# DTolm/VkFFT

Measured on AMD Instinct MI355X. Metric: GFLOP/s (5N log2 N) + achieved HBM GB/s, batched 1D C2C fp32, 1/2/4/8 GPU, higher is better.
Workload: dtype f32; 1 GPU; batched 1D C2C fp32 in-place, N=2^8..2^22, batch=2^27/N (1 GiB per GPU), FFT+iFFT pair per size per step (sample-0 protocol); buffer_bytes_per_gpu=1073741824, parallelism=batch-sharded x1, no collectives

## Files before the change

### vkfft_amd/csrc/kernel_pow2_pk.h

```cpp
#pragma once
#include "kernel_pow2_lean.h"
#include <utility>

namespace vkfft_mi355x {

#if defined(VKFFT_HOSTEMU)
template <typename T> struct pk2 { T x, y; };
template <typename T> inline pk2<T> operator+(pk2<T> a, pk2<T> b) { return {a.x + b.x, a.y + b.y}; }
template <typename T> inline pk2<T> operator-(pk2<T> a, pk2<T> b) { return {a.x - b.x, a.y - b.y}; }
template <typename T> inline pk2<T> operator*(pk2<T> a, pk2<T> b) { return {a.x * b.x, a.y * b.y}; }
template <typename T> inline pk2<T> operator-(pk2<T> a) { return {-a.x, -a.y}; }
template <typename V> inline V pk_xx(V a) { return V{a.x, a.x}; }
template <typename V> inline V pk_yy(V a) { return V{a.y, a.y}; }
#define VKFFT_PIN2(x) do { } while (0)
#else
template <typename T> struct pk2_of;
template <> struct pk2_of<float> { typedef float type __attribute__((ext_vector_type(2))); };
template <> struct pk2_of<double> { typedef double type __attribute__((ext_vector_type(2))); };
template <typename T> using pk2 = typename pk2_of<T>::type;
template <typename V> __device__ inline V pk_xx(V a) { return __builtin_shufflevector(a, a, 0, 0); }
template <typename V> __device__ inline V pk_yy(V a) { return __builtin_shufflevector(a, a, 1, 1); }
#define VKFFT_PIN2(x) asm volatile("" : "+v"(x))
#endif
template <typename T> __host__ __device__ inline pk2<T> pk_splat(T s) { return pk2<T>{s, s}; }

#if defined(VKFFT_HOSTEMU)
#define VKFFT_PKPROF_DECL do { } while (0)
#define VKFFT_PKPROF(i) do { } while (0)
#define VKFFT_PKPROF_FLUSH() do { } while (0)
#else
#define VKFFT_PKPROF_DECL __shared__ unsigned long long spc[12]; unsigned long long ptk = 0; if constexpr ((MODE & 4) != 0) { if (threadIdx.x < 12) spc[threadIdx.x] = 0; ptk = __builtin_readcyclecounter(); }
#define VKFFT_PKPROF(i) do { if constexpr ((MODE & 4) != 0) { if (threadIdx.x == 0) { const unsigned long long now = __builtin_readcyclecounter(); spc[i] += now - ptk; ptk = now; } } } while (0)
#define VKFFT_PKPROF_FLUSH() do { if constexpr ((MODE & 4) != 0) { if (threadIdx.x == 0 && p.prof) { for (int i = 0; i < 12; i++) p.prof[(size_t)blockIdx.x * 12 + i] = spc[i]; } } } while (0)
#endif

template <typename T> struct cxp { pk2<T> re, im; };
template <typename T> __device__ inline cxp<T> pcadd(cxp<T> a, cxp<T> b) { return {a.re + b.re, a.im + b.im}; }
template <typename T> __device__ inline cxp<T> pcsub(cxp<T> a, cxp<T> b) { return {a.re - b.re, a.im - b.im}; }
template <typename T> __device__ inline cxp<T> pcmul1(cxp<T> a, pk2<T> w) {
	const pk2<T> wx = pk_xx(w), wy = pk_yy(w);
	return {a.re * wx - a.im * wy, a.re * wy + a.im * wx};
}
template <typename T> __device__ inline cxp<T> pcmul2(cxp<T> a, pk2<T> wre, pk2<T> wim) { return {a.re * wre - a.im * wim, a.re * wim + a.im * wre}; }

#if defined(VKFFT_HOSTEMU)
template <typename T> inline pk2<T> pk_cmul_aos(pk2<T> a, pk2<T> b) { return {a.x * b.x - a.y * b.y, a.x * b.y + a.y * b.x}; }
#else
template <typename T> __device__ inline pk2<T> pk_cmul_aos(pk2<T> a, pk2<T> b) {
	const pk2<T> br = __builtin_shufflevector(b, -b, 3, 0);
	return pk_xx(a) * b + pk_yy(a) * br;
}
#endif

template <int R, typename T> __device__ inline void pk_dif_inplace(cxp<T>* x) {
#pragma unroll
	for (int h = R / 2; h >= 1; h >>= 1) {
#pragma unroll
		for (int blk = 0; blk < R; blk += 2 * h) {
#pragma unroll
			for (int j = 0; j < h; j++) {
				const cxp<T> a = x[blk + j], b = x[blk + j + h];
				x[blk + j] = pcadd(a, b);
				const int kk = j * (16 / h);
				if (kk == 0) x[blk + j + h] = pcsub(a, b);
				else if (kk == 8) x[blk + j + h] = cxp<T>{a.im - b.im, b.re - a.re};
				else {
					const cxp<T> d = pcsub(a, b);
					const pk2<T> c = pk_splat<T>((T)pow2_cos32(kk)), s = pk_splat<T>((T)pow2_sin32(kk));
					x[blk + j + h] = cxp<T>{d.re * c + d.im * s, d.im * c - d.re * s};
				}
			}
		}
		VKFFT_SCHED_FENCE();
	}
}

template <typename T, typename TW> __device__ inline pk2<T> pk_tw(const TW& lut, uint32_t s, uint32_t constOff) { const cx<T> w = lut.get(s, constOff); return pk2<T>{w.x, w.y}; }

template <typename T, typename SCH, int SI, int TPF, typename TW, int TWG>
__device__ inline void pk_lean_butterflies(cxp<T>* v, const TW lut, const uint32_t tau) {
	constexpr int LOGE = SCH::LOGE, E = 1 << LOGE;
	constexpr int LOGR = SCH::bits[SI], R = 1 << LOGR, NB = E / R;
	constexpr int LOGS = SCH::logS(SI), S = 1 << LOGS;
#pragma unroll
	for (int b = 0; b < NB; b++) {
		if constexpr (SI > 0) {
			const uint32_t s = (tau + b * TPF) & (S - 1);
			constexpr int LO = SCH::lutOff(SI);
#pragma unroll
			for (int i0 = 1; i0 < R; i0 += TWG) {
				const int i1 = i0 + TWG < R ? i0 + TWG : R;
				pk2<T> w[TWG];
#pragma unroll
				for (int i = i0; i < i1; i++) w[i - i0] = pk_tw<T>(lut, s, (uint32_t)(LO + (i - 1) * S));
				VKFFT_SCHED_FENCE();
#pragma unroll
				for (int i = i0; i < i1; i++) { cxp<T>& q = v[b + i * NB]; q = pcmul1(q, w[i - i0]); VKFFT_PIN2(q.re); VKFFT_PIN2(q.im); }
				VKFFT_SCHED_FENCE();
			}
		}
		cxp<T> x[R];
#pragma unroll
		for (int i = 0; i < R; i++) x[i] = v[b + i * NB];
		pk_dif_inplace<R, T>(x);
#pragma unroll
		for (int k = 0; k < R; k++) v[b + k * NB] = x[pow2_bitrev(k, LOGR)];
	}
}

template <typename T, typename SCH, int SI, int TPF, int TC, int PART>
__device__ inline void pk_lean_exchange_part(cxp<T>* v, T* plane, const uint32_t tau) {
	constexpr int LOGE = SCH::LOGE, E = 1 << LOGE, P = SCH::bits[0];
	constexpr int LOGR = SCH::bits[SI], R = 1 << LOGR, NB = E / R;
	constexpr int LOGS = SCH::logS(SI), S = 1 << LOGS;
	static_assert(TC > 0 && TC % 2 == 0, "column tiles of even width");
#pragma unroll
	for (int b = 0; b < NB; b++) {
		const uint32_t t = tau + b * TPF;
		const uint32_t s = t & (S - 1);
		const uint32_t ob = ((t - s) << LOGR) + s;
		T* const wp = plane + pow2_lean_slot<TC, P>(ob);
#pragma unroll
		for (int k = 0; k < R; k++) *(pk2<T>*)(wp + pow2_lean_step<TC, P>(k * S)) = PART ? v[b + k * NB].im : v[b + k * NB].re;
	}
	VKFFT_SYNC();
	const T* const rp = plane + pow2_lean_slot<TC, P>(tau);
#pragma unroll
	for (int m = 0; m < E; m++) {
		const pk2<T> r = *(const pk2<T>*)(rp + pow2_lean_step<TC, P>(m * TPF));
		if (PART) v[m].im = r; else v[m].re = r;
	}
}

template <typename T, typename SCH, int SI, int TPF, int TC, typename TW, int TWG>
__device__ inline void pk_lean_stages(cxp<T>* v, T* plane, const TW lut, const uint32_t tau) {
	pk_lean_butterflies<T, SCH, SI, TPF, TW, TWG>(v, lut, tau);
	if constexpr (SI + 1 < SCH::NS) {
		pk_lean_exchange_part<T, SCH, SI, TPF, TC, 0>(v, plane, tau);
		VKFFT_SYNC();
		pk_lean_exchange_part<T, SCH, SI, TPF, TC, 1>(v, plane, tau);
		if constexpr (SI + 2 < SCH::NS) VKFFT_SYNC();
		pk_lean_stages<T, SCH, SI + 1, TPF, TC, TW, TWG>(v, plane, lut, tau);
	}
}

template <typename T, int L, int E, int TPF, int TC, int NT>
__device__ inline void pk_lean_transpose(const cxp<T>* v, cxp<T>* r, T* plane, const uint32_t tid, const uint32_t c, const uint32_t tau) {
	constexpr int PT = L + 64 / TC;
	static_assert(E * NT * 2 == L * TC && (PT % 2) == 0, "two columns per thread");
#pragma unroll
	for (int part = 0; part < 2; part++) {
		if (part) VKFFT_SYNC();
		T* const w0 = plane + c * PT + tau;
#pragma unroll
		for (int m = 0; m < E; m++) { const pk2<T> q = part ? v[m].im : v[m].re; w0[m * TPF] = q.x; w0[PT + m * TPF] = q.y; }
		VKFFT_SYNC();
#pragma unroll
		for (int i = 0; i < E; i++) {
			const uint32_t idx = tid + i * NT;
			const uint32_t kp = idx % (L / 2), cc = idx / (L / 2);
			const pk2<T> pr = *(const pk2<T>*)(plane + cc * PT + 2u * kp);
			if (part) r[i].im = pr; else r[i].re = pr;
		}
	}
}

#if defined(VKFFT_HOSTEMU)
template <typename T> struct pk4 { T x, y, z, w; };
template <typename T, int AUX> inline pk4<T> gb_load_aos2(GBuf b, uint32_t voff, uint32_t soff) {
	if (voff >= kGbRange) return pk4<T>{(T)0, (T)0, (T)0, (T)0};
	const T* q = (const T*)(b.base + (uint64_t)voff + soff);
	return pk4<T>{q[0], q[1], q[2], q[3]};
}
template <typename T> inline cxp<T> pk_from_aos(pk4<T> t) { return cxp<T>{{t.x, t.z}, {t.y, t.w}}; }
template <typename T, int AUX> inline void gb_store_aos2(GBuf b, uint32_t voff, cxp<T> v) {
	if (voff >= kGbRange) return;
	T* q = (T*)(b.base + (uint64_t)voff);
	q[0] = v.re.x; q[1] = v.im.x; q[2] = v.re.y; q[3] = v.im.y;
}
template <typename T, int E> inline void gb_landed_raw(pk4<T>*) { }
template <typename T, int AUX> inline cxp<T> gb_load_soa2(GBuf b, uint32_t voff, uint32_t soff) {
	if (voff >= kGbRange) return cxp<T>{{(T)0, (T)0}, {(T)0, (T)0}};
	const T* q = (const T*)(b.base + (uint64_t)voff + soff);
	return cxp<T>{{q[0], q[1]}, {q[2], q[3]}};
}
template <typename T, int AUX> inline void gb_store_soa2(GBuf b, uint32_t voff, cxp<T> v) {
	if (voff >= kGbRange) return;
	T* q = (T*)(b.base + (uint64_t)voff);
	q[0] = v.re.x; q[1] = v.re.y; q[2] = v.im.x; q[3] = v.im.y;
}
template <typename T, int E> inline void gb_landed_pk(cxp<T>*) { }
#else
template <typename T> struct pk4_of;
template <> struct pk4_of<float> { typedef float type __attribute__((ext_vector_type(4))); };
template <typename T> using pk4 = typename pk4_of<T>::type;
template <typename T, int AUX> __device__ inline pk4<T> gb_load_aos2(GBuf b, uint32_t voff, uint32_t soff) {
	static_assert(sizeof(T) == 4, "pairs of fp32 complex only");
	return __builtin_bit_cast(pk4<T>, __builtin_amdgcn_raw_buffer_load_b128(b.r, voff, soff, AUX));
}
template <typename T> __device__ inline cxp<T> pk_from_aos(pk4<T> t) {
	T a = t.y, b = t.z;
	asm("v_swap_b32 %0, %1" : "+v"(a), "+v"(b));
	return cxp<T>{pk2<T>{t.x, a}, pk2<T>{b, t.w}};
}
template <typename T, int AUX> __device__ inline void gb_store_aos2(GBuf b, uint32_t voff, cxp<T> v) {
	static_assert(sizeof(T) == 4, "pairs of fp32 complex only");
	T a = v.re.y, c = v.im.x;
	asm("v_swap_b32 %0, %1" : "+v"(a), "+v"(c));
	const pk4<T> t = {v.re.x, a, c, v.im.y};
	__builtin_amdgcn_raw_buffer_store_b128(__builtin_bit_cast(vk_u32x4, t), b.r, voff, 0, AUX);
}
template <typename T, int E> __device__ inline void gb_landed_raw(pk4<T>* v) {
#pragma unroll
	for (int m = 0; m < E; m++) asm volatile("" : "+v"(v[m]));
}
template <typename T, int AUX> __device__ inline cxp<T> gb_load_soa2(GBuf b, uint32_t voff, uint32_t soff) {
	static_assert(sizeof(T) == 4, "pairs of fp32 complex only");
	const vk_u32x4 t = __builtin_amdgcn_raw_buffer_load_b128(b.r, voff, soff, AUX);
	return cxp<T>{pk2<T>{__uint_as_float(t.x), __uint_as_float(t.y)}, pk2<T>{__uint_as_float(t.z), __uint_as_float(t.w)}};
}
template <typename T, int AUX> __device__ inline void gb_store_soa2(GBuf b, uint32_t voff, cxp<T> v) {
	static_assert(sizeof(T) == 4, "pairs of fp32 complex only");
	vk_u32x4 t; t.x = __float_as_uint(v.re.x); t.y = __float_as_uint(v.re.y); t.z = __float_as_uint(v.im.x); t.w = __float_as_uint(v.im.y);
	__builtin_amdgcn_raw_buffer_store_b128(t, b.r, voff, 0, AUX);
}
template <typename T, int E> __device__ inline void gb_landed_pk(cxp<T>* v) {
#pragma unroll
	for (int m = 0; m < E; m++) asm volatile("" : "+v"(v[m].re), "+v"(v[m].im));
}
#endif

template <typename T> struct RowGlobal {
	GBuf tab;
	__device__ inline cxp<T> get(uint32_t tau, uint32_t constK) const { return gb_load_soa2<T, 0>(tab, tau * 16u, constK * 16u); }
};
template <typename T> struct RowLds {
	const cx<T>* tab;
	__device__ inline cxp<T> get(uint32_t tau, uint32_t constK) const {
#if defined(VKFFT_HOSTEMU)
		const T* q = (const T*)(tab + 2u * (tau + constK));
		return cxp<T>{{q[0], q[1]}, {q[2], q[3]}};
#else
		const pk4<T> t = *(const pk4<T>*)(tab + 2u * (tau + constK));
		return cxp<T>{pk2<T>{t.x, t.y}, pk2<T>{t.z, t.w}};
#endif
	}
};
template <typename T, int LOGE> struct PkFsTw {
	static constexpr int HIB = (LOGE + 1) / 2, LOB = LOGE - HIB, NA = 1 << HIB, NB = (1 << LOB) - 1;
	pk2<T> lo[NA + NB], hi[NA + NB];
};
template <typename T, int LOGE, int TPF>
__device__ inline void pk_fs_request(PkFsTw<T, LOGE>& q, const GBuf gtab, const uint32_t fsLoBits, const uint32_t tau, const uint32_t colEven) {
	constexpr uint32_t ES = (uint32_t)sizeof(cx<T>);
	constexpr int LOB = PkFsTw<T, LOGE>::LOB, NA = PkFsTw<T, LOGE>::NA, NB = PkFsTw<T, LOGE>::NB;
	const uint32_t loMask = (1u << fsLoBits) - 1u;
	const uint32_t hiBase = (loMask + 1u) * ES;
	auto ld = [&](uint32_t voff, uint32_t soff) { const cx<T> w = gb_load<T>(gtab, voff, soff); return pk2<T>{w.x, w.y}; };
#pragma unroll
	for (int j = 0; j < NA + NB; j++) {
		const uint32_t e = (j < NA ? tau + (uint32_t)((j << LOB) * TPF) : (uint32_t)((j - NA + 1) * TPF)) * colEven;
		q.lo[j] = ld((e & loMask) * ES, 0); q.hi[j] = ld((e >> fsLoBits) * ES, hiBase);
	}
}
template <typename T, int LOGE, int TPF, typename ROW>
__device__ inline void pk_fs_apply(cxp<T>* v, const PkFsTw<T, LOGE>& q, const ROW row, const uint32_t tau, const pk2<T>* hiStep = nullptr) {
	constexpr int E = 1 << LOGE;
	constexpr int LOB = PkFsTw<T, LOGE>::LOB, NA = PkFsTw<T, LOGE>::NA, NB = PkFsTw<T, LOGE>::NB;
	pk2<T> A[NA], B[NB + 1];
#pragma unroll
	for (int j = 0; j < NA; j++) { A[j] = pk_cmul_aos<T>(q.lo[j], q.hi[j]); if (hiStep) A[j] = pk_cmul_aos<T>(A[j], *hiStep); }
	B[0] = pk2<T>{(T)1, (T)0};
#pragma unroll
	for (int i = 1; i <= NB; i++) B[i] = pk_cmul_aos<T>(q.lo[NA + i - 1], q.hi[NA + i - 1]);
	constexpr int CH = 4;
#pragma unroll
	for (int m0 = 0; m0 < E; m0 += CH) {
		cxp<T> uv[CH];
#pragma unroll
		for (int i = 0; i < CH; i++) uv[i] = row.get(tau, (uint32_t)((m0 + i) * TPF));
		VKFFT_SCHED_FENCE();
#pragma unroll
		for (int i = 0; i < CH; i++) {
			const int m = m0 + i;
			const pk2<T> w0 = (m & ((1 << LOB) - 1)) ? pk_cmul_aos<T>(A[m >> LOB], B[m & ((1 << LOB) - 1)]) : A[m >> LOB];
			const pk2<T> w0x = pk_xx(w0), w0y = pk_yy(w0);
			v[m] = pcmul2(v[m], w0x * uv[i].re - w0y * uv[i].im, w0y * uv[i].re + w0x * uv[i].im);
			VKFFT_PIN2(v[m].re); VKFFT_PIN2(v[m].im);
		}
		VKFFT_SCHED_FENCE();
	}
}

#if defined(VKFFT_HOSTEMU)
template <typename T> inline pk2<T> pka_cmul(pk2<T> a, pk2<T> w) { return {a.x * w.x - a.y * w.y, a.y * w.x + a.x * w.y}; }
template <typename T> inline pk2<T> pka_cmul_const(pk2<T> d, T c, T s) { return {d.x * c + d.y * s, d.y * c - d.x * s}; }
template <typename T> inline pk2<T> pka_sub_mi(pk2<T> a, pk2<T> b) { return {a.y - b.y, b.x - a.x}; }
#else
template <typename T> __device__ inline pk2<T> pka_cmul(pk2<T> a, pk2<T> w) {
	if constexpr (sizeof(T) == 4) {
		const pk2<T> t = a * pk_xx(w);
		pk2<T> r;
		asm("v_pk_fma_f32 %0, %1, %2, %3 op_sel:[1,1,0] op_sel_hi:[0,1,1] neg_lo:[1,0,0]" : "=v"(r) : "v"(a), "v"(w), "v"(t));
		return r;
	} else return pk2<T>{a.x * w.x - a.y * w.y, a.y * w.x + a.x * w.y};
}
template <typename T> __device__ inline pk2<T> pka_cmul_const(pk2<T> d, T c, T s) {
	if constexpr (sizeof(T) == 4) {
		const pk2<T> t = d * pk_splat<T>(c), ss = pk_splat<T>(s);
		pk2<T> r;
		asm("v_pk_fma_f32 %0, %1, %2, %3 op_sel:[1,0,0] op_sel_hi:[0,1,1] neg_hi:[1,0,0]" : "=v"(r) : "v"(d), "s"(ss), "v"(t));
		return r;
	} else return pk2<T>{d.x * c + d.y * s, d.y * c - d.x * s};
}
template <typename T> __device__ inline pk2<T> pka_sub_mi(pk2<T> a, pk2<T> b) {
	if constexpr (sizeof(T) == 4) {
		pk2<T> r;
		asm("v_pk_add_f32 %0, %1, %2 op_sel:[1,1] op_sel_hi:[0,0] neg_lo:[0,1] neg_hi:[1,0]" : "=v"(r) : "v"(a), "v"(b));
		return r;
	} else return pk2<T>{a.y - b.y, b.x - a.x};
}
#endif

template <typename F, int... I> __host__ __device__ inline void vk_static_for_impl(F&& f, std::integer_sequence<int, I...>) { (f(std::integral_constant<int, I>{}), ...); }
template <int N, typename F> __host__ __device__ inline void vk_static_for(F&& f) { vk_static_for_impl(f, std::make_integer_sequence<int, N>{}); }
constexpr int vk_ilog2(int n) { int l = 0; while ((1 << l) < n) l++; return l; }

template <int R, typename T> __device__ inline void pka_dif_inplace(pk2<T>* x) {
	vk_static_for<vk_ilog2(R)>([&](auto li) {
		constexpr int h = (R / 2) >> decltype(li)::value;
		vk_static_for<R / 2>([&](auto bi) {
			constexpr int blk = (decltype(bi)::value / h) * 2 * h, j = decltype(bi)::value % h;
			const pk2<T> a = x[blk + j], b = x[blk + j + h];
			x[blk + j] = a + b;
			constexpr int kk = j * (16 / h);
			if constexpr (kk == 0) x[blk + j + h] = a - b;
			else if constexpr (kk == 8) x[blk + j + h] = pka_sub_mi<T>(a, b);
			else x[blk + j + h] = pka_cmul_const<T>(a - b, (T)pow2_cos32(kk), (T)pow2_sin32(kk));
		});
		VKFFT_SCHED_FENCE();
	});
}

template <typename T, typename SCH, int SI, int TPF, typename TW, int TWG>
__device__ inline void pka_lean_butterflies(pk2<T>* v, const TW lut, const uint32_t tau) {
	constexpr int LOGE = SCH::LOGE, E = 1 << LOGE;
	constexpr int LOGR = SCH::bits[SI], R = 1 << LOGR, NB = E / R;
	constexpr int LOGS = SCH::logS(SI), S = 1 << LOGS;
#pragma unroll
	for (int b = 0; b < NB; b++) {
		if constexpr (SI > 0) {
			const uint32_t s = (tau + b * TPF) & (S - 1);
			constexpr int LO = SCH::lutOff(SI);
#pragma unroll
			for (int i0 = 1; i0 < R; i0 += TWG) {
				const int i1 = i0 + TWG < R ? i0 + TWG : R;
				pk2<T> w[TWG];
#pragma unroll
				for (int i = i0; i < i1; i++) w[i - i0] = pk_tw<T>(lut, s, (uint32_t)(LO + (i - 1) * S));
				VKFFT_SCHED_FENCE();
#pragma unroll
				for (int i = i0; i < i1; i++) { pk2<T>& q = v[b + i * NB]; q = pka_cmul<T>(q, w[i - i0]); VKFFT_PIN2(q); }
				VKFFT_SCHED_FENCE();
			}
		}
		pk2<T> x[R];
#pragma unroll
		for (int i = 0; i < R; i++) x[i] = v[b + i * NB];
		pka_dif_inplace<R, T>(x);
#pragma unroll
		for (int k = 0; k < R; k++) v[b + k * NB] = x[pow2_bitrev(k, LOGR)];
	}
}
template <typename T, typename SCH, int SI, int TPF, int PART, bool WAVE>
__device__ inline void pka_lean_exchange_part(pk2<T>* v, T* plane, const uint32_t tau) {
	constexpr int LOGE = SCH::LOGE, E = 1 << LOGE, P = SCH::bits[0];
	constexpr int LOGR = SCH::bits[SI], R = 1 << LOGR, NB = E / R;
	constexpr int LOGS = SCH::logS(SI), S = 1 << LOGS;
#pragma unroll
	for (int b = 0; b < NB; b++) {
		const uint32_t t = tau + b * TPF;
		const uint32_t s = t & (S - 1);
		const uint32_t ob = ((t - s) << LOGR) + s;
		T* const wp = plane + pow2_lean_slot<0, P>(ob);
#pragma unroll
		for (int k = 0; k < R; k++) wp[pow2_lean_step<0, P>(k * S)] = PART ? v[b + k * NB].y : v[b + k * NB].x;
	}
	if constexpr (WAVE) VKFFT_WAVE_SYNC(); else VKFFT_SYNC();
	const T* const rp = plane + pow2_lean_slot<0, P>(tau);
#pragma unroll
	for (int m = 0; m < E; m++) {
		const T r = rp[pow2_lean_step<0, P>(m * TPF)];
		if (PART) v[m].y = r; else v[m].x = r;
	}
}
template <typename T, typename SCH, int SI, int TPF, typename TW, int TWG, bool WAVE = false>
__device__ inline void pka_lean_stages(pk2<T>* v, T* plane, const TW lut, const uint32_t tau) {
	pka_lean_butterflies<T, SCH, SI, TPF, TW, TWG>(v, lut, tau);
	if constexpr (SI + 1 < SCH::NS) {
		pka_lean_exchange_part<T, SCH, SI, TPF, 0, WAVE>(v, plane, tau);
		if constexpr (WAVE) VKFFT_WAVE_SYNC(); else VKFFT_SYNC();
		pka_lean_exchange_part<T, SCH, SI, TPF, 1, WAVE>(v, plane, tau);
		if constexpr (SI + 2 < SCH::NS) { if constexpr (WAVE) VKFFT_WAVE_SYNC(); else VKFFT_SYNC(); }
		pka_lean_stages<T, SCH, SI + 1, TPF, TW, TWG, WAVE>(v, plane, lut, tau);
	}
}

template <typename T, typename SCH, int WPE, int TWG, int FPW = 1>
__global__ void __launch_bounds__(((1 << SCH::LOGN) >> SCH::LOGE) * FPW, WPE) pow2_row_lean_pk_kernel(const PassParams p) {
	constexpr int LOGN = SCH::LOGN, N = 1 << LOGN, LOGE = SCH::LOGE, E = 1 << LOGE, TPF = N / E;
	constexpr uint32_t ES = (uint32_t)sizeof(cx<T>);
	constexpr int PL = (int)pow2_lean_plane_elems<SCH, 0>();
	__shared__ T planes[FPW * PL];
	const uint32_t tau = FPW > 1 ? threadIdx.x % (uint32_t)TPF : threadIdx.x, fl = FPW > 1 ? threadIdx.x / (uint32_t)TPF : 0u;
	T* const plane = planes + fl * PL;
	uint32_t wg = p.reverseTiles ? gridDim.x - 1u - blockIdx.x : blockIdx.x;
	const uint32_t f0 = (wg % p.tilesPerG0) * (uint32_t)FPW + fl;
	wg /= p.tilesPerG0;
	const uint32_t g1 = wg % p.dim[1].count, g2 = wg / p.dim[1].count;
	const bool valid = FPW == 1 || f0 < p.dim[0].count;
	const GBuf gin = make_gbuf((const cx<T>*)p.in + ((int64_t)g1 * p.dim[1].inStride + (int64_t)g2 * p.dim[2].inStride + (int64_t)(FPW == 1 ? f0 : f0 - fl) * p.dim[0].inStride));
	const GBuf gout = make_gbuf((cx<T>*)p.out + ((int64_t)g1 * p.dim[1].outStride + (int64_t)g2 * p.dim[2].outStride + (int64_t)(FPW == 1 ? f0 : f0 - fl) * p.dim[0].outStride));
	const GBuf glut = make_gbuf(p.lut);
	const uint32_t laneIn = !valid ? kGbInvalid : (tau + (FPW == 1 ? 0u : fl * (uint32_t)p.dim[0].inStride)) * ES;
	const uint32_t laneOut = !valid ? kGbInvalid : (tau + (FPW == 1 ? 0u : fl * (uint32_t)p.dim[0].outStride)) * ES;
	pk2<T> v[E];
	auto ld = [&](uint32_t voff, uint32_t soff) { const cx<T> q = gb_load<T>(gin, voff, soff); return pk2<T>{q.x, q.y}; };
	if (p.padInN) {
#pragma unroll
		for (int m = 0; m < E; m++) v[m] = ld((tau + (uint32_t)(m * TPF) - p.padInL < p.padInN) ? kGbInvalid : laneIn, (uint32_t)(m * TPF) * ES);
	} else {
#pragma unroll
		for (int m = 0; m < E; m++) v[m] = ld(laneIn, (uint32_t)(m * TPF) * ES);
	}
	if (p.swapIn) {
#pragma unroll
		for (int m = 0; m < E; m++) v[m].y = -v[m].y;
	}
	pka_lean_stages<T, SCH, 0, TPF, TwGlobal<T>, TWG, false>(v, plane, TwGlobal<T>{glut}, tau);
	const T sc = (T)p.scale;
	if (sc != (T)1 || p.swapOut) {
		const pk2<T> f = {sc, p.swapOut ? -sc : sc};
#pragma unroll
		for (int m = 0; m < E; m++) v[m] = v[m] * f;
	}
	if (p.padOutN) {
#pragma unroll
		for (int m = 0; m < E; m++) gb_store<T>(gout, (tau + (uint32_t)(m * TPF) - p.padOutL < p.padOutN) ? kGbInvalid : laneOut, (uint32_t)(m * TPF) * ES, cx<T>{v[m].x, v[m].y});
	} else {
#pragma unroll
		for (int m = 0; m < E; m++) gb_store<T>(gout, laneOut, (uint32_t)(m * TPF) * ES, cx<T>{v[m].x, v[m].y});
	}
}
template <typename T, typename SCH, int WPE, int TWG, int FPW = 1> void pow2_row_lean_pk_launch(const PassParams& prm, dim3 grid, hipStream_t s) {
	hipLaunchKernelGGL((pow2_row_lean_pk_kernel<T, SCH, WPE, TWG, FPW>), grid, dim3(((1 << SCH::LOGN) >> SCH::LOGE) * FPW), 0, s, prm);
}

template <typename T, typename SCH, int TWG>
__global__ void __launch_bounds__((1 << SCH::LOGN) >> SCH::LOGE, 2) pow2_row_pairs_kernel(const PassParams p) {
	constexpr int LOGN2 = SCH::LOGN, N2 = 1 << LOGN2, LOGE = SCH::LOGE, E = 1 << LOGE, TPF = N2 / E, H = E / 2;
	constexpr uint32_t ES = (uint32_t)sizeof(cx<T>);
	typedef Pow2Sched<SCH::bits[0], SCH::bits[1], SCH::bits[2], 1> SF;
	constexpr int LUTC = SF::lutOff(3);
	static_assert(SCH::bits[3] == 0 && sizeof(T) == 4, "three stages on pairs of fp32 samples");
	__shared__ __attribute__((aligned(16))) T plane[pow2_lean_plane_elems<SCH, 2>()];
	const uint32_t tau = threadIdx.x;
	const uint32_t total = p.tilesPerG0 * p.dim[1].count * p.dim[2].count;
	const GBuf glut = make_gbuf(p.lut);
	pk4<T> ra[H], rb[H];
	auto rowBase = [&](uint32_t w, bool out) -> int64_t {
		uint32_t wg = p.reverseTiles ? total - 1u - w : w;
		const uint32_t f0 = wg % p.tilesPerG0; wg /= p.tilesPerG0;
		const uint32_t g1 = wg % p.dim[1].count, g2 = wg / p.dim[1].count;
		return out ? (int64_t)g1 * p.dim[1].outStride + (int64_t)g2 * p.dim[2].outStride + (int64_t)f0 * p.dim[0].outStride
		           : (int64_t)g1 * p.dim[1].inStride + (int64_t)g2 * p.dim[2].inStride + (int64_t)f0 * p.dim[0].inStride;
	};
	auto request = [&](uint32_t w, int h, pk4<T>* raw) {
		VKFFT_OPAQUE_ZERO(oq);
		const bool live = w < total;
		const GBuf gin = make_gbuf((const cx<T>*)p.in + (live ? rowBase(w, false) : 0));
		const uint32_t lane = live ? tau * 2u * ES + oq : kGbInvalid;
#pragma unroll
		for (int m = 0; m < H; m++) raw[m] = gb_load_aos2<T, 0>(gin, lane, (uint32_t)((h * H + m) * TPF) * 2u * ES);
	};
	uint32_t w = blockIdx.x;
	request(w, 0, ra);
	request(w, 1, rb);
	for (; w < total; w += gridDim.x) {
		cxp<T> v[E];
#pragma unroll
		for (int m = 0; m < H; m++) v[m] = pk_from_aos<T>(ra[m]);
#pragma unroll
		for (int m = 0; m < H; m++) v[H + m] = pk_from_aos<T>(rb[m]);
		if (p.swapIn) {
#pragma unroll
			for (int m = 0; m < E; m++) v[m].im = -v[m].im;
		}
		request(w + gridDim.x, 0, ra);
		pk_lean_stages<T, SCH, 0, TPF, 2, TwGlobal<T>, TWG>(v, plane, TwGlobal<T>{glut}, tau);
		VKFFT_SYNC();
		const T sc = (T)p.scale, sci = p.swapOut ? -sc : sc;
		const GBuf gout = make_gbuf((cx<T>*)p.out + rowBase(w, true));
		VKFFT_OPAQUE_ZERO(oz);
		const uint32_t lane = tau * ES + oz;
		constexpr int CH = 8;
#pragma unroll
		for (int m0 = 0; m0 < E; m0 += CH) {
			pk2<T> tw[CH];
#pragma unroll
			for (int i = 0; i < CH; i++) tw[i] = pk_tw<T>(TwGlobal<T>{glut}, tau, (uint32_t)(LUTC + (m0 + i) * TPF));
			VKFFT_SCHED_FENCE();
#pragma unroll
			for (int i = 0; i < CH; i++) {
				const int m = m0 + i;
				const T tr = v[m].re.y * tw[i].x - v[m].im.y * tw[i].y, ti = v[m].re.y * tw[i].y + v[m].im.y * tw[i].x;
				const cx<T> lo = {(v[m].re.x + tr) * sc, (v[m].im.x + ti) * sci}, hi = {(v[m].re.x - tr) * sc, (v[m].im.x - ti) * sci};
				gb_store<T>(gout, lane, (uint32_t)(m * TPF) * ES, lo);
				gb_store<T>(gout, lane, (uint32_t)(m * TPF + N2) * ES, hi);
			}
			VKFFT_SCHED_FENCE();
		}
		request(w + gridDim.x, 1, rb);
	}
}
template <typename T, typename SCH, int TWG> void pow2_row_pairs_launch(const PassParams& prm, dim3 grid, hipStream_t s) {
	const unsigned resident = pow2_num_cus();
	hipLaunchKernelGGL((pow2_row_pairs_kernel<T, SCH, TWG>), dim3(grid.x < resident ? grid.x : resident), dim3((1 << SCH::LOGN) >> SCH::LOGE), 0, s, prm);
}

}
```

### vkfft_amd/csrc/kernels_pow2.hip

```cpp
#include "engine.h"
#include "kernel_pow2.h"
#include "kernel_pow2_pk.h"
#include <cstdio>
#include <cstdlib>

namespace vkfft_mi355x {


template <typename T, typename SCH, int FPW> void pow2_row_launch(const PassParams& prm, dim3 grid, hipStream_t s) {
	constexpr int threads = ((1 << SCH::LOGN) >> SCH::LOGE) * FPW;
	hipLaunchKernelGGL((pow2_row_kernel<T, SCH, FPW>), grid, dim3(threads), 0, s, prm);
}

template <typename T, typename SCH, int TC> void pow2_col_launch(const PassParams& prm, dim3 grid, hipStream_t s) {
	constexpr int threads = ((1 << SCH::LOGN) >> SCH::LOGE) * TC;
	if (prm.bigSpan) hipLaunchKernelGGL((pow2_col_kernel<T, SCH, TC, true>), grid, dim3(threads), 0, s, prm);
	else hipLaunchKernelGGL((pow2_col_kernel<T, SCH, TC, false>), grid, dim3(threads), 0, s, prm);
}

#define VKFFT_P2C(T, dp, b0, b1, b2, b3, tc) \
	{ (b0) + (b1) + (b2) + (b3), dp, {b0, b1, b2, b3}, tc, (((1 << ((b0) + (b1) + (b2) + (b3))) >> Pow2Sched<b0, b1, b2, b3>::LOGE) * (tc)), &pow2_col_launch<T, Pow2Sched<b0, b1, b2, b3>, tc> }

#define VKFFT_P2(T, dp, b0, b1, b2, b3, fpw) \
	{ (b0) + (b1) + (b2) + (b3), dp, {b0, b1, b2, b3}, fpw, (((1 << ((b0) + (b1) + (b2) + (b3))) >> Pow2Sched<b0, b1, b2, b3>::LOGE) * (fpw)), &pow2_row_launch<T, Pow2Sched<b0, b1, b2, b3>, fpw> }

#define VKFFT_P2L(T, dp, b0, b1, b2, b3, wpe, twg, pfn) \
	{ (b0) + (b1) + (b2) + (b3), dp, {b0, b1, b2, b3}, 1, ((1 << ((b0) + (b1) + (b2) + (b3))) >> Pow2Sched<b0, b1, b2, b3>::LOGE), &pow2_row_lean_launch<T, Pow2Sched<b0, b1, b2, b3>, wpe, twg, pfn>, "pow2_row_lean_kernel" }

#define VKFFT_P2K(T, dp, b0, b1, b2, b3, wpe, twg) \
	{ (b0) + (b1) + (b2) + (b3), dp, {b0, b1, b2, b3}, 1, ((1 << ((b0) + (b1) + (b2) + (b3))) >> Pow2Sched<b0, b1, b2, b3>::LOGE), &pow2_row_lean_pk_launch<T, Pow2Sched<b0, b1, b2, b3>, wpe, twg>, "pow2_row_lean_pk_kernel" }

#define VKFFT_P2KF(T, dp, b0, b1, b2, b3, wpe, twg, fpw) \
	{ (b0) + (b1) + (b2) + (b3), dp, {b0, b1, b2, b3}, fpw, ((1 << ((b0) + (b1) + (b2) + (b3))) >> Pow2Sched<b0, b1, b2, b3>::LOGE) * (fpw), &pow2_row_lean_pk_launch<T, Pow2Sched<b0, b1, b2, b3>, wpe, twg, fpw>, "pow2_row_lean_pk_kernel" }

#define VKFFT_P2R(T, dp, b0, b1, b2, twg) \
	{ (b0) + (b1) + (b2) + 1, dp, {b0, b1, b2, 1}, 1, ((1 << ((b0) + (b1) + (b2))) >> Pow2Sched<b0, b1, b2, 0>::LOGE), &pow2_row_pairs_launch<T, Pow2Sched<b0, b1, b2, 0>, twg>, "pow2_row_pairs_kernel", true }

static const Pow2Variant kPow2Variants[] = {
	VKFFT_P2(float, false, 2, 0, 0, 0, 64),
	VKFFT_P2(float, false, 3, 0, 0, 0, 64),
	VKFFT_P2(float, false, 4, 0, 0, 0, 64),
	VKFFT_P2(float, false, 3, 2, 0, 0, 32),
	VKFFT_P2(float, false, 3, 3, 0, 0, 32),
	VKFFT_P2(float, false, 4, 3, 0, 0, 16),
	VKFFT_P2(float, false, 4, 4, 0, 0, 8),
	VKFFT_P2KF(float, false, 5, 4, 0, 0, 4, 16, 16), VKFFT_P2(float, false, 5, 4, 0, 0, 8),
	VKFFT_P2KF(float, false, 5, 5, 0, 0, 4, 16, 8), VKFFT_P2(float, false, 5, 5, 0, 0, 8),
	VKFFT_P2KF(float, false, 4, 4, 3, 0, 5, 16, 4), VKFFT_P2(float, false, 5, 5, 1, 0, 2),
	VKFFT_P2KF(float, false, 4, 4, 4, 0, 5, 16, 1), VKFFT_P2(float, false, 4, 4, 4, 0, 1),
	VKFFT_P2K(float, false, 5, 4, 4, 0, 4, 16), VKFFT_P2(float, false, 5, 4, 4, 0, 1), VKFFT_P2L(float, false, 5, 4, 4, 0, 4, 16, 0),
	VKFFT_P2K(float, false, 5, 5, 4, 0, 4, 16), VKFFT_P2(float, false, 5, 5, 4, 0, 1), VKFFT_P2L(float, false, 5, 5, 4, 0, 4, 16, 0),
	VKFFT_P2R(float, false, 5, 5, 4, 8), VKFFT_P2K(float, false, 5, 5, 5, 0, 4, 16), VKFFT_P2L(float, false, 5, 5, 5, 0, 4, 16, 0),
	VKFFT_P2(double, true, 2, 0, 0, 0, 64),
	VKFFT_P2(double, true, 3, 0, 0, 0, 64),
	VKFFT_P2(double, true, 4, 0, 0, 0, 64),
	VKFFT_P2(double, true, 3, 2, 0, 0, 32),
	VKFFT_P2(double, true, 3, 3, 0, 0, 32),
	VKFFT_P2(double, true, 3, 2, 2, 0, 16),
	VKFFT_P2(double, true, 3, 3, 2, 0, 8),
	VKFFT_P2(double, true, 3, 3, 3, 0, 4),
	VKFFT_P2(double, true, 3, 3, 2, 2, 2), VKFFT_P2(double, true, 4, 3, 3, 0, 2),
	VKFFT_P2(double, true, 3, 3, 3, 2, 1), VKFFT_P2(double, true, 4, 4, 3, 0, 1),
	VKFFT_P2(double, true, 3, 3, 3, 3, 1), VKFFT_P2(double, true, 4, 4, 4, 0, 1),
	VKFFT_P2(double, true, 4, 3, 3, 3, 1),
};
constexpr int kNumPow2Variants = (int)(sizeof(kPow2Variants) / sizeof(kPow2Variants[0]));

static const Pow2Variant kPow2ColVariants[] = {
	VKFFT_P2C(float, false, 1, 0, 0, 0, 64), VKFFT_P2C(float, false, 2, 0, 0, 0, 64), VKFFT_P2C(float, false, 3, 0, 0, 0, 64),
	VKFFT_P2C(float, false, 2, 2, 0, 0, 32), VKFFT_P2C(float, false, 2, 2, 0, 0, 16),
	VKFFT_P2C(float, false, 3, 2, 0, 0, 32), VKFFT_P2C(float, false, 3, 2, 0, 0, 16),
	VKFFT_P2C(float, false, 3, 3, 0, 0, 32), VKFFT_P2C(float, false, 3, 3, 0, 0, 16),
	VKFFT_P2C(float, false, 4, 3, 0, 0, 32), VKFFT_P2C(float, false, 4, 3, 0, 0, 16), VKFFT_P2C(float, false, 3, 2, 2, 0, 32),
	VKFFT_P2C(float, false, 4, 4, 0, 0, 32), VKFFT_P2C(float, false, 4, 4, 0, 0, 16), VKFFT_P2C(float, false, 3, 3, 2, 0, 32), VKFFT_P2C(float, false, 3, 3, 2, 0, 16), VKFFT_P2C(float, false, 5, 3, 0, 0, 32),
	VKFFT_P2C(float, false, 5, 4, 0, 0, 32), VKFFT_P2C(float, false, 4, 3, 2, 0, 16), VKFFT_P2C(float, false, 4, 3, 2, 0, 32), VKFFT_P2C(float, false, 3, 3, 3, 0, 16), VKFFT_P2C(float, false, 5, 4, 0, 0, 16),
	VKFFT_P2C(float, false, 5, 5, 0, 0, 16), VKFFT_P2C(float, false, 4, 3, 3, 0, 16), VKFFT_P2C(float, false, 4, 3, 3, 0, 8),
	VKFFT_P2C(double, true, 1, 0, 0, 0, 32), VKFFT_P2C(double, true, 2, 0, 0, 0, 32), VKFFT_P2C(double, true, 3, 0, 0, 0, 32),
	VKFFT_P2C(double, true, 2, 2, 0, 0, 16),
	VKFFT_P2C(double, true, 3, 2, 0, 0, 16),
	VKFFT_P2C(double, true, 3, 3, 0, 0, 16),
	VKFFT_P2C(double, true, 3, 2, 2, 0, 16), VKFFT_P2C(double, true, 4, 3, 0, 0, 16),
	VKFFT_P2C(double, true, 3, 3, 2, 0, 16), VKFFT_P2C(double, true, 4, 4, 0, 0, 16),
	VKFFT_P2C(double, true, 3, 3, 3, 0, 8), VKFFT_P2C(double, true, 4, 3, 2, 0, 8), VKFFT_P2C(double, true, 3, 3, 3, 0, 16),
	VKFFT_P2C(double, true, 4, 3, 3, 0, 8),
};
constexpr int kNumPow2ColVariants = (int)(sizeof(kPow2ColVariants) / sizeof(kPow2ColVariants[0]));

template <typename T, typename SCH, int FPW> void pow2_blue_launch(const PassParams& prm, dim3 grid, hipStream_t s) {
	constexpr int threads = ((1 << SCH::LOGN) >> SCH::LOGE) * FPW;
	const unsigned resident = pow2_num_cus() * 8u;
	hipLaunchKernelGGL((pow2_blue_kernel<T, SCH, FPW>), dim3(grid.x < resident ? grid.x : resident), dim3(threads), 0, s, prm);
}
#define VKFFT_P2B(T, dp, b0, b1, b2, b3, fpw) \
	{ (b0) + (b1) + (b2) + (b3), dp, {b0, b1, b2, b3}, fpw, (((1 << ((b0) + (b1) + (b2) + (b3))) >> Pow2Sched<b0, b1, b2, b3>::LOGE) * (fpw)), &pow2_blue_launch<T, Pow2Sched<b0, b1, b2, b3>, fpw> }
static const Pow2Variant kPow2BlueVariants[] = {
	VKFFT_P2B(float, false, 3, 3, 0, 0, 32),
	VKFFT_P2B(float, false, 4, 3, 0, 0, 16),
	VKFFT_P2B(float, false, 4, 4, 0, 0, 16),
	VKFFT_P2B(float, false, 4, 3, 2, 0, 8),
	VKFFT_P2B(float, false, 4, 3, 3, 0, 4),
	VKFFT_P2B(float, false, 4, 4, 3, 0, 2),
	VKFFT_P2B(float, false, 4, 4, 4, 0, 1),
	VKFFT_P2B(float, false, 4, 3, 3, 3, 1),
	VKFFT_P2B(float, false, 4, 4, 3, 3, 1),
	VKFFT_P2B(double, true, 3, 3, 0, 0, 32),
	VKFFT_P2B(double, true, 3, 2, 2, 0, 16),
	VKFFT_P2B(double, true, 3, 3, 2, 0, 8),
	VKFFT_P2B(double, true, 3, 3, 3, 0, 4),
	VKFFT_P2B(double, true, 3, 3, 2, 2, 2),
	VKFFT_P2B(double, true, 3, 3, 3, 2, 1),
	VKFFT_P2B(double, true, 3, 3, 3, 3, 1),
	VKFFT_P2B(double, true, 4, 3, 3, 3, 1),
};
constexpr int kNumPow2BlueVariants = (int)(sizeof(kPow2BlueVariants) / sizeof(kPow2BlueVariants[0]));

template <typename T, typename SCH, int TC, int MODE> void pow2_col_blue_launch(const PassParams& prm, dim3 grid, hipStream_t s) {
	constexpr int threads = ((1 << SCH::LOGN) >> SCH::LOGE) * TC;
	hipLaunchKernelGGL((pow2_col_blue_kernel<T, SCH, TC, MODE>), grid, dim3(threads), 0, s, prm);
}
struct Pow2ColBlueVariant { Pow2Variant v; int mode; };
#define VKFFT_P2CB1(T, dp, b0, b1, b2, b3, tc, mode) \
	{ { (b0) + (b1) + (b2) + (b3), dp, {b0, b1, b2, b3}, tc, (((1 << ((b0) + (b1) + (b2) + (b3))) >> Pow2Sched<b0, b1, b2, b3>::LOGE) * (tc)), &pow2_col_blue_launch<T, Pow2Sched<b0, b1, b2, b3>, tc, mode> }, mode }
#define VKFFT_P2CB(T, dp, b0, b1, b2, b3, tc) VKFFT_P2CB1(T, dp, b0, b1, b2, b3, tc, 1), VKFFT_P2CB1(T, dp, b0, b1, b2, b3, tc, 2), VKFFT_P2CB1(T, dp, b0, b1, b2, b3, tc, 3), VKFFT_P2CB1(T, dp, b0, b1, b2, b3, tc, 4), \
	VKFFT_P2CB1(T, dp, b0, b1, b2, b3, tc, 5), VKFFT_P2CB1(T, dp, b0, b1, b2, b3, tc, 6), VKFFT_P2CB1(T, dp, b0, b1, b2, b3, tc, 8)
static const Pow2ColBlueVariant kPow2ColBlueVariants[] = {
	VKFFT_P2CB(float, false, 3, 3, 0, 0, 32),
	VKFFT_P2CB(float, false, 4, 3, 0, 0, 32),
	VKFFT_P2CB(float, false, 4, 4, 0, 0, 32),
	VKFFT_P2CB(float, false, 4, 3, 2, 0, 16),
	VKFFT_P2CB(float, false, 4, 3, 3, 0, 16),
	VKFFT_P2CB1(float, false, 4, 4, 3, 0, 8, 5),
	VKFFT_P2CB1(float, false, 4, 3, 3, 0, 8, 7),
	VKFFT_P2CB1(double, true, 3, 3, 3, 0, 8, 7),
	VKFFT_P2CB(double, true, 3, 3, 0, 0, 16),
	VKFFT_P2CB(double, true, 3, 2, 2, 0, 16),
	VKFFT_P2CB(double, true, 3, 3, 2, 0, 16),
	VKFFT_P2CB(double, true, 3, 3, 3, 0, 8),
	VKFFT_P2CB(double, true, 4, 3, 3, 0, 8),
};
constexpr int kNumPow2ColBlueVariants = (int)(sizeof(kPow2ColBlueVariants) / sizeof(kPow2ColBlueVariants[0]));

int launch_pow2_col_blue(const PassPlan& pp, const PassParams& prm, hipStream_t stream) {
	const uint64_t grid64 = (uint64_t)prm.tilesPerG0 * prm.dim[1].count * prm.dim[2].count;
	if (grid64 == 0) return 0;
	if (grid64 > 0x7fffffffull || pp.variant < 0 || pp.variant >= kNumPow2ColBlueVariants) return 4039;
	kPow2ColBlueVariants[pp.variant].v.launch(prm, dim3((uint32_t)grid64), stream);
	return hipGetLastError() == hipSuccess ? 0 : 4039;
}

int launch_pow2_blue(const PassPlan& pp, const PassParams& prm, hipStream_t stream) {
	const uint64_t grid64 = (uint64_t)prm.tilesPerG0 * prm.dim[1].count * prm.dim[2].count;
	if (grid64 == 0) return 0;
	if (grid64 > 0x7fffffffull || pp.variant < 0 || pp.variant >= kNumPow2BlueVariants) return 4039;
	kPow2BlueVariants[pp.variant].launch(prm, dim3((uint32_t)grid64), stream);
	return hipGetLastError() == hipSuccess ? 0 : 4039;
}

const char* pow2_row_kernel_name(int variant) {
	if (variant < 0 || variant >= kNumPow2Variants || !kPow2Variants[variant].name) return "pow2_row_kernel";
	return kPow2Variants[variant].name;
}

int launch_pow2(const PassPlan& pp, const PassParams& prm, hipStream_t stream) {
	const uint64_t grid64 = (uint64_t)prm.tilesPerG0 * (prm.colMerge ? 1u : prm.dim[1].count) * prm.dim[2].count;
	if (grid64 == 0) return 0;
	const bool col = pp.kernel == KERNEL_POW2_COL;
	if (grid64 > 0x7fffffffull || pp.variant < 0 || pp.variant >= (col ? kNumPow2ColVariants : kNumPow2Variants)) return 4039;
	(col ? kPow2ColVariants : kPow2Variants)[pp.variant].launch(prm, dim3((uint32_t)grid64), stream);
	return hipGetLastError() == hipSuccess ? 0 : 4039;
}


static bool pow2_lookup(const Pow2Variant* tab, int ntab, int want, uint32_t log2n, bool dp, int* variant, int bits[4], int* fpw, int* threads, bool padded = false) {
	const int found = pick_variant(ntab, want, [&](int i) { return tab[i].log2n != (int)log2n || tab[i].dp != dp ? 0 : padded && tab[i].noPadMasks ? 2 : 1; });
	if (found < 0) return false;
	*variant = found;
	for (int k = 0; k < 4; k++) bits[k] = tab[found].bits[k];
	*fpw = tab[found].fpw; *threads = tab[found].threads;
	return true;
}
bool pow2_row_lookup(uint32_t log2n, bool dp, int want, int* variant, int bits[4], int* fpw, int* threads, bool padded) {
	return pow2_lookup(kPow2Variants, kNumPow2Variants, want, log2n, dp, variant, bits, fpw, threads, padded);
}
bool pow2_col_lookup(uint32_t log2n, bool dp, int want, int* variant, int bits[4], int* tc, int* threads) {
	return pow2_lookup(kPow2ColVariants, kNumPow2ColVariants, want, log2n, dp, variant, bits, tc, threads);
}

bool pow2_col_blue_lookup(uint32_t log2l, bool dp, int mode, int* variant, int bits[4], int* tc, int* threads) {
	for (int i = 0; i < kNumPow2ColBlueVariants; i++) {
		const Pow2ColBlueVariant& e = kPow2ColBlueVariants[i];
		if (e.v.log2n != (int)log2l || e.v.dp != dp || e.mode != mode) continue;
		*variant = i;
		for (int k = 0; k < 4; k++) bits[k] = e.v.bits[k];
		*tc = e.v.fpw; *threads = e.v.threads;
		return true;
	}
	return false;
}
bool pow2_blue_lookup(uint32_t log2m, bool dp, int want, int* variant, int bits[4], int* fpw, int* threads) {
	return pow2_lookup(kPow2BlueVariants, kNumPow2BlueVariants, want, log2m, dp, variant, bits, fpw, threads);
}


}
```

Measured before the change: 19780 GFLOP/s.

## Pair lanes via DPP for 16-byte stores in row-pairs kernel and add variants

The final radix-2 butterfly of the pairs kernel now swaps values between adjacent lanes with DPP quad permutes. Each lane can then write two consecutive complex outputs with one wide store instead of two scattered 8-byte stores. Loads and stores take a cache-policy (aux) parameter set to 2. The launch bound and persistent grid size now scale with an LDS/register-derived workgroups-per-CU estimate, and new pairs variants are registered for 2^13 and 2^14. The cost is extra cross-lane permutes and a sign multiply per output, and the occupancy estimate could raise register pressure.

```diff
diff --git a/vkfft_amd/csrc/kernel_pow2_pk.h b/vkfft_amd/csrc/kernel_pow2_pk.h
--- a/vkfft_amd/csrc/kernel_pow2_pk.h
+++ b/vkfft_amd/csrc/kernel_pow2_pk.h
@@ -456,13 +456,42 @@
 	hipLaunchKernelGGL((pow2_row_lean_pk_kernel<T, SCH, WPE, TWG, FPW>), grid, dim3(((1 << SCH::LOGN) >> SCH::LOGE) * FPW), 0, s, prm);
 }
 
-template <typename T, typename SCH, int TWG>
-__global__ void __launch_bounds__((1 << SCH::LOGN) >> SCH::LOGE, 2) pow2_row_pairs_kernel(const PassParams p) {
+
+#if defined(VKFFT_HOSTEMU)
+template <typename T> inline void pk_pair_bcast4(const T (&x)[4], T (&e)[4], T (&o)[4]) {
+	__shared__ T slot[1024][4];
+	const uint32_t t = threadIdx.x;
+	for (int i = 0; i < 4; i++) slot[t][i] = x[i];
+	VKFFT_WAVE_SYNC();
+	for (int i = 0; i < 4; i++) { e[i] = slot[t & ~1u][i]; o[i] = slot[t | 1u][i]; }
+	VKFFT_WAVE_SYNC();
+}
+#else
+template <typename T> __device__ inline void pk_pair_bcast4(const T (&x)[4], T (&e)[4], T (&o)[4]) {
+	static_assert(sizeof(T) == 4, "pairs of fp32 complex only");
+#pragma unroll
+	for (int i = 0; i < 4; i++) {
+		const int xi = __builtin_bit_cast(int, x[i]);
+		e[i] = __builtin_bit_cast(T, __builtin_amdgcn_update_dpp(xi, xi, 0xA0, 0xF, 0xF, false));
+		o[i] = __builtin_bit_cast(T, __builtin_amdgcn_update_dpp(xi, xi, 0xF5, 0xF, 0xF, false));
+	}
+}
+#endif
+
+template <typename T, typename SCH> constexpr int pow2_row_pairs_wg_per_cu() {
+	constexpr int E = 1 << SCH::LOGE, NT = (1 << SCH::LOGN) >> SCH::LOGE;
+	constexpr int byLds = (160 * 1024) / (int)(pow2_lean_plane_elems<SCH, 2>() * sizeof(T));
+	constexpr int byRegs = (2048 / (8 * E)) * 64 / NT;
+	return byLds < byRegs ? (byLds < 1 ? 1 : byLds) : (byRegs < 1 ? 1 : byRegs);
+}
+
+template <typename T, typename SCH, int TWG, int AUX>
+__global__ void __launch_bounds__((1 << SCH::LOGN) >> SCH::LOGE, (pow2_row_pairs_wg_per_cu<T, SCH>() * ((1 << SCH::LOGN) >> SCH::LOGE) + 255) / 256) pow2_row_pairs_kernel(const PassParams p) {
 	constexpr int LOGN2 = SCH::LOGN, N2 = 1 << LOGN2, LOGE = SCH::LOGE, E = 1 << LOGE, TPF = N2 / E, H = E / 2;
 	constexpr uint32_t ES = (uint32_t)sizeof(cx<T>);
 	typedef Pow2Sched<SCH::bits[0], SCH::bits[1], SCH::bits[2], 1> SF;
 	constexpr int LUTC = SF::lutOff(3);
-	static_assert(SCH::bits[3] == 0 && sizeof(T) == 4, "three stages on pairs of fp32 samples");
+	static_assert(SCH::bits[3] == 0 && sizeof(T) == 4 && TPF % 64 == 0, "three stages on pairs of fp32 samples; lane pairs inside a wavefront");
 	__shared__ __attribute__((aligned(16))) T plane[pow2_lean_plane_elems<SCH, 2>()];
 	const uint32_t tau = threadIdx.x;
 	const uint32_t total = p.tilesPerG0 * p.dim[1].count * p.dim[2].count;
@@ -481,7 +510,7 @@
 		const GBuf gin = make_gbuf((const cx<T>*)p.in + (live ? rowBase(w, false) : 0));
 		const uint32_t lane = live ? tau * 2u * ES + oq : kGbInvalid;
 #pragma unroll
-		for (int m = 0; m < H; m++) raw[m] = gb_load_aos2<T, 0>(gin, lane, (uint32_t)((h * H + m) * TPF) * 2u * ES);
+		for (int m = 0; m < H; m++) raw[m] = gb_load_aos2<T, AUX>(gin, lane, (uint32_t)((h * H + m) * TPF) * 2u * ES);
 	};
 	uint32_t w = blockIdx.x;
 	request(w, 0, ra);
@@ -502,7 +531,9 @@
 		const T sc = (T)p.scale, sci = p.swapOut ? -sc : sc;
 		const GBuf gout = make_gbuf((cx<T>*)p.out + rowBase(w, true));
 		VKFFT_OPAQUE_ZERO(oz);
-		const uint32_t lane = tau * ES + oz;
+		const bool odd = ((tau + oz) & 1u) != 0;
+		const T sgn = odd ? (T)-1 : (T)1;
+		const uint32_t lane = (odd ? tau - 1u + (uint32_t)N2 : tau) * ES + oz;
 		constexpr int CH = 8;
 #pragma unroll
 		for (int m0 = 0; m0 < E; m0 += CH) {
@@ -514,18 +545,20 @@
 			for (int i = 0; i < CH; i++) {
 				const int m = m0 + i;
 				const T tr = v[m].re.y * tw[i].x - v[m].im.y * tw[i].y, ti = v[m].re.y * tw[i].y + v[m].im.y * tw[i].x;
-				const cx<T> lo = {(v[m].re.x + tr) * sc, (v[m].im.x + ti) * sci}, hi = {(v[m].re.x - tr) * sc, (v[m].im.x - ti) * sci};
-				gb_store<T>(gout, lane, (uint32_t)(m * TPF) * ES, lo);
-				gb_store<T>(gout, lane, (uint32_t)(m * TPF + N2) * ES, hi);
+				const T x[4] = {v[m].re.x, v[m].im.x, tr, ti};
+				T e[4], o[4];
+				pk_pair_bcast4<T>(x, e, o);
+				const cx<T> s0 = {(e[0] + sgn * e[2]) * sc, (e[1] + sgn * e[3]) * sci}, s1 = {(o[0] + sgn * o[2]) * sc, (o[1] + sgn * o[3]) * sci};
+				gb_store2_x<T, AUX>(gout, lane + (uint32_t)(m * TPF) * ES, s0, s1);
 			}
 			VKFFT_SCHED_FENCE();
 		}
 		request(w + gridDim.x, 1, rb);
 	}
 }
-template <typename T, typename SCH, int TWG> void pow2_row_pairs_launch(const PassParams& prm, dim3 grid, hipStream_t s) {
-	const unsigned resident = pow2_num_cus();
-	hipLaunchKernelGGL((pow2_row_pairs_kernel<T, SCH, TWG>), dim3(grid.x < resident ? grid.x : resident), dim3((1 << SCH::LOGN) >> SCH::LOGE), 0, s, prm);
-}
-
-}
+template <typename T, typename SCH, int TWG, int AUX> void pow2_row_pairs_launch(const PassParams& prm, dim3 grid, hipStream_t s) {
+	const unsigned resident = pow2_num_cus() * (unsigned)pow2_row_pairs_wg_per_cu<T, SCH>();
+	hipLaunchKernelGGL((pow2_row_pairs_kernel<T, SCH, TWG, AUX>), dim3(grid.x < resident ? grid.x : resident), dim3((1 << SCH::LOGN) >> SCH::LOGE), 0, s, prm);
+}
+
+}
diff --git a/vkfft_amd/csrc/kernels_pow2.hip b/vkfft_amd/csrc/kernels_pow2.hip
--- a/vkfft_amd/csrc/kernels_pow2.hip
+++ b/vkfft_amd/csrc/kernels_pow2.hip
@@ -33,8 +33,8 @@
 #define VKFFT_P2KF(T, dp, b0, b1, b2, b3, wpe, twg, fpw) \
 	{ (b0) + (b1) + (b2) + (b3), dp, {b0, b1, b2, b3}, fpw, ((1 << ((b0) + (b1) + (b2) + (b3))) >> Pow2Sched<b0, b1, b2, b3>::LOGE) * (fpw), &pow2_row_lean_pk_launch<T, Pow2Sched<b0, b1, b2, b3>, wpe, twg, fpw>, "pow2_row_lean_pk_kernel" }
 
-#define VKFFT_P2R(T, dp, b0, b1, b2, twg) \
-	{ (b0) + (b1) + (b2) + 1, dp, {b0, b1, b2, 1}, 1, ((1 << ((b0) + (b1) + (b2))) >> Pow2Sched<b0, b1, b2, 0>::LOGE), &pow2_row_pairs_launch<T, Pow2Sched<b0, b1, b2, 0>, twg>, "pow2_row_pairs_kernel", true }
+#define VKFFT_P2R(T, dp, b0, b1, b2, twg, aux) \
+	{ (b0) + (b1) + (b2) + 1, dp, {b0, b1, b2, 1}, 1, ((1 << ((b0) + (b1) + (b2))) >> Pow2Sched<b0, b1, b2, 0>::LOGE), &pow2_row_pairs_launch<T, Pow2Sched<b0, b1, b2, 0>, twg, aux>, "pow2_row_pairs_kernel", true }
 
 static const Pow2Variant kPow2Variants[] = {
 	VKFFT_P2(float, false, 2, 0, 0, 0, 64),
@@ -48,9 +48,9 @@
 	VKFFT_P2KF(float, false, 5, 5, 0, 0, 4, 16, 8), VKFFT_P2(float, false, 5, 5, 0, 0, 8),
 	VKFFT_P2KF(float, false, 4, 4, 3, 0, 5, 16, 4), VKFFT_P2(float, false, 5, 5, 1, 0, 2),
 	VKFFT_P2KF(float, false, 4, 4, 4, 0, 5, 16, 1), VKFFT_P2(float, false, 4, 4, 4, 0, 1),
-	VKFFT_P2K(float, false, 5, 4, 4, 0, 4, 16), VKFFT_P2(float, false, 5, 4, 4, 0, 1), VKFFT_P2L(float, false, 5, 4, 4, 0, 4, 16, 0),
-	VKFFT_P2K(float, false, 5, 5, 4, 0, 4, 16), VKFFT_P2(float, false, 5, 5, 4, 0, 1), VKFFT_P2L(float, false, 5, 5, 4, 0, 4, 16, 0),
-	VKFFT_P2R(float, false, 5, 5, 4, 8), VKFFT_P2K(float, false, 5, 5, 5, 0, 4, 16), VKFFT_P2L(float, false, 5, 5, 5, 0, 4, 16, 0),
+	VKFFT_P2R(float, false, 5, 4, 3, 8, 2), VKFFT_P2K(float, false, 5, 4, 4, 0, 4, 16), VKFFT_P2(float, false, 5, 4, 4, 0, 1), VKFFT_P2L(float, false, 5, 4, 4, 0, 4, 16, 0),
+	VKFFT_P2K(float, false, 5, 5, 4, 0, 4, 16), VKFFT_P2(float, false, 5, 5, 4, 0, 1), VKFFT_P2L(float, false, 5, 5, 4, 0, 4, 16, 0), VKFFT_P2R(float, false, 5, 4, 4, 8, 2),
+	VKFFT_P2R(float, false, 5, 5, 4, 8, 2), VKFFT_P2K(float, false, 5, 5, 5, 0, 4, 16), VKFFT_P2L(float, false, 5, 5, 5, 0, 4, 16, 0),
 	VKFFT_P2(double, true, 2, 0, 0, 0, 64),
 	VKFFT_P2(double, true, 3, 0, 0, 0, 64),
 	VKFFT_P2(double, true, 4, 0, 0, 0, 64),
```

New measurement: 19830 GFLOP/s (median of 6 runs). About the same (+0.2%).
